# k-sheridan/mantis

Measured on AMD Instinct MI355X. Metric: poses/sec + p50 per-frame latency, 1280x720 4-cam batch, higher is better.
Workload: dtype f64; 1 GPU; config3: 4-cam 1280x720 rig, shared map, full mantis3 path per camera + joint rig Gauss-Newton; cams_per_rig=4, contexts_per_gpu=6, landmarks=720, parallelism=rig-data-parallel x1

## Files before the change

mantis_amd/csrc/api.hip:

```cpp
#include <hip/hip_runtime.h>
#ifndef MK_FC_THREADS
#define MK_FC_THREADS 256
#endif

#include <algorithm>
#include <atomic>
#include <cfloat>
#include <chrono>
#include <cmath>
#include <cstdio>
#include <cstdlib>
#include <cstring>
#include <mutex>
#include <sstream>
#include <string>
#include <thread>
#include <vector>

#include <rccl/rccl.h>

#include "kernels.hip"

using namespace mk;

// ... 66 lines not shown
      return MANTIS_ERR_DEVICE;                                                   \
    }                                                                             \
  } while (0)

struct Ctx {
  mantis_config cfg{};
  hipStream_t s = nullptr;
  hipStream_t s_copy = nullptr;
  hipEvent_t ev_gauss = nullptr;
  hipEvent_t ev_wait = nullptr;
  int spin_frames = 16;
  std::string err;
  uint64_t rng_state = 1;
  double* d_lm = nullptr;
  int nw = 0, nr = 0, ng = 0;
  int F = 0, Wmax = 0, Hmax = 0;
  int n_cu = 256;
  bool trace_lds_ok = false;
  size_t trace_lds_max = 0;
  int trace_lds_frames = 0;
  int fc_small_frames = 0;
  size_t plane = 0;
  int pool_cap = 0;
  uint16_t* d_lroot = nullptr;
  size_t lstride = 0;
  size_t fstride = 0;
  uint8_t *d_bgr = nullptr, *d_strong = nullptr, *d_edge = nullptr,
          *d_det = nullptr, *d_mask = nullptr;
  int32_t* d_lab = nullptr;
  uint32_t *d_eb = nullptr, *d_b1 = nullptr, *d_b2 = nullptr;
// ... 83 lines not shown
  int gauss_cap = 0;
  RigWJob* d_rwjobs = nullptr;
  double* d_rwout = nullptr;
  size_t rw_cap = 0;
  int rw_rigs = 0, rw_C = 0;
  std::vector<double> rw_weights, rw_c2w, rw_sums;
  std::vector<int32_t> rw_chosen;
  bool has_prior = false;
  double prior_Twb[16];
  double* d_markov = nullptr;
  MarkovOp* d_mops = nullptr;
  int markov_n = 0;
  int32_t* d_agree = nullptr;
  bool agreed_fail = false;
  struct CallGraph {
    int n = 0, W = 0, H = 0, live = 0, nw = 0, nr = 0, ng = 0;
    bool vec = false;
    const void* lm = nullptr;
    const void* gauss = nullptr;
    hipGraphExec_t pre = nullptr, post = nullptr;
  };
  std::vector<CallGraph> graphs;
  bool use_graphs = false;
  bool screen_off = false;
  std::vector<std::pair<Cam, ScreenCam>> scam_cache;
  struct Track {
    void* d_in = nullptr;
    void* h_in = nullptr;
    size_t in_cap = 0;
    void* d_state = nullptr;
    void* d_res = nullptr;
// ... 62 lines not shown
  const bool mismatch = v[1] != -v[2];
  c->agreed_fail = v[0] != 0 || mismatch;
  if (local != MANTIS_OK) return local;
  if (v[0]) {
    c->err = "another rank of the communicator failed before this exchange (see its mantis_last_error)";
    return MANTIS_ERR_COMM;
  }
  if (mismatch) {
    c->err = "ranks passed different frame counts to a batched exchange (every rank must pass the same n_frames)";
    return MANTIS_ERR_ARG;
  }
  return MANTIS_OK;
}

inline Landmarks lmk_of(const Ctx* c) {
  return Landmarks{c->d_lm, c->nw, c->nr, c->ng, c->d_lm ? (const float4*)(c->d_lm + kLmfOffset) : nullptr};
}

void mark(Ctx* c, const char* name) {
  if (!c->prof) return;
  if (c->ev.size() <= c->ev_names.size()) {
    hipEvent_t e;
    (void)hipEventCreate(&e);
    c->ev.push_back(e);
  }
  (void)hipEventRecord(c->ev[c->ev_names.size()], c->s);
  c->ev_names.push_back(name);
}

struct Ctx;
hipError_t wait_stream(Ctx* c, int frames);
// ... 440 lines not shown
  if (ei != hipSuccess) {
    *out = nullptr;
    c->err = std::string("hipGraphInstantiate: ") + hipGetErrorString(ei);
    return MANTIS_ERR_DEVICE;
  }
  return MANTIS_OK;
}

Ctx::CallGraph* call_graph(Ctx* c, int n, int W, int H, const Shard* sh) {
  if (!c->use_graphs || sh || c->prof || n > c->fc_small_frames) return nullptr;
  const size_t hr_lds = (size_t)((H + HR_ROWS - 1) / HR_ROWS) * HR_ROWS * bits::words(W) * sizeof(uint32_t);
  if (!(c->hyst_rec && bits::words(W) <= 63 && H <= HR_ROWS * HR_MAXW && hr_lds <= c->hyst_rec_lds)) return nullptr;
  const int live = std::max(1, g_live_ctx[c->cfg.device & 63].load());
  for (auto& g : c->graphs)
    if (g.n == n && g.W == W && g.H == H && g.vec == c->vec_ok && g.live == live && g.lm == c->d_lm &&
        g.nw == c->nw && g.nr == c->nr && g.ng == c->ng && g.gauss == c->d_gauss)
      return &g;
  if (c->graphs.size() >= 8) {
    if (c->graphs.front().pre) (void)hipGraphExecDestroy(c->graphs.front().pre);
    if (c->graphs.front().post) (void)hipGraphExecDestroy(c->graphs.front().post);
    c->graphs.erase(c->graphs.begin());
  }
  Ctx::CallGraph g;
  g.n = n; g.W = W; g.H = H; g.vec = c->vec_ok; g.live = live;
  g.lm = c->d_lm; g.nw = c->nw; g.nr = c->nr; g.ng = c->ng; g.gauss = c->d_gauss;
  c->graphs.push_back(g);
  return &c->graphs.back();
}

mantis_status process_frames(Ctx* c, const mantis_image* cams, int n, const Shard* sh = nullptr) {
  if (!c->d_lm) { c->err = "map not set (mantis_set_map)"; return MANTIS_ERR_STATE; }
  if (n <= 0 || n > c->F) { c->err = "frame count exceeds max_cams"; return MANTIS_ERR_ARG; }
  const int ng = sh ? sh->n_global : n;
  if ((int64_t)c->cfg.particles * c->cfg.iterations * 6 * ng > INT32_MAX) {
    c->err = "particles x iterations x 6 x frames (all rig cameras when sharded) exceeds 2^31 gaussians per call";
    return MANTIS_ERR_ARG;
  }
  if (mantis_status e = ensure_gauss(c, ng)) return e;
  struct Joiner {
    std::thread t;
// ... 410 lines not shown

mantis_status mantis_set_map(void* ctx, const double* white, int32_t nw, const double* red, int32_t nr,
                             const double* green, int32_t ng) {
  Ctx* c = (Ctx*)ctx;
  if (c) bind_device(c);
  if (!c || nw < 0 || nr < 0 || ng < 0 || nw + nr + ng > 768 || ng > 64 || (nw && !white) || (nr && !red) ||
      (ng && !green)) {
    if (c) c->err = "map: need nw+nr+ng <= 768 and ng <= 64";
    return MANTIS_ERR_ARG;
  }
  std::vector<double> all;
  all.insert(all.end(), white, white + 3 * nw);
  all.insert(all.end(), red, red + 3 * nr);
  all.insert(all.end(), green, green + 3 * ng);
  const size_t nl = (size_t)nw + nr + ng;
  std::vector<double> buf(kLmfOffset + 2 * 768, 0.0);
  std::copy(all.begin(), all.end(), buf.begin());
  float* lf = (float*)(buf.data() + kLmfOffset);
  for (size_t i = 0; i < nl; i++) screen_landmark(all.data() + 3 * i, lf + 4 * i);
  if (c->d_lm) (void)hipFree(c->d_lm);
  c->d_lm = nullptr;
  if (dalloc(c, &c->d_lm, buf.size()) != MANTIS_OK) return MANTIS_ERR_OOM;
  HIP_OK(hipMemcpy(c->d_lm, buf.data(), sizeof(double) * buf.size(), hipMemcpyHostToDevice));
  c->nw = nw;
  c->nr = nr;
  c->ng = ng;
  c->h_lm = all;
  c->rf.pitch = 0;
  c->rf.rigs = 0;
  return MANTIS_OK;
}

int32_t mantis_parse_coordinates(const char* s, double* xyz, int32_t max_pts) {
  if (!s) return 0;
  std::vector<std::string> rows;
  std::stringstream ts(s);
  std::string tmp;
  while (std::getline(ts, tmp, ';')) {
    tmp.erase(std::remove(tmp.begin(), tmp.end(), '\n'), tmp.end());
    tmp.erase(std::remove(tmp.begin(), tmp.end(), ' '), tmp.end());
    rows.push_back(tmp);
// ... 766 lines not shown
```

mantis_amd/csrc/hostcheck.cpp:

```cpp
#include <algorithm>
#include <cstdint>
#include <cstring>
#include <vector>

static int g_jacobi_ff = 1;
#define MK_JACOBI_FF g_jacobi_ff
#include "mk_bits.h"
#include "mk_contour.h"
#include "mk_gn.h"
#include "mk_math.h"
#include "mk_mcl.h"
#include "mk_mcl_color.h"
#include "mk_mcl_modes.h"
#include "mk_refine.h"
#include "mk_rpp.h"
#include "mk_screen.h"
#include "mk_shard.h"
#include "mk_sort.h"
#include "mk_track.h"

extern "C" {

void hc_set_jacobi_ff(int on) { g_jacobi_ff = on; }

// ... 264 lines not shown
    const bool in = rp[2] > 0 && mk::in_frame(u, v, H, W);
    float xl[4];
    mk::screen_landmark(X + 3 * i, xl);
    int px = 0, py = 0;
    const int st = mk::screen_project(mk::posef_from(T), xl[0], xl[1], xl[2], xl[3], sc, W, H, &px, &py);
    res[4 * i] = st;
    res[4 * i + 1] = in;
    res[4 * i + 2] = st == mk::SCR_IN ? px : (in ? mk::cv_round(u) : 0);
    res[4 * i + 3] = st == mk::SCR_IN ? py : (in ? mk::cv_round(v) : 0);
    if ((st == mk::SCR_IN && (!in || px != mk::cv_round(u) || py != mk::cv_round(v))) || (st == mk::SCR_OUT && in))
      bad++;
  }
  return bad;
}

int hc_sizeof_cam_result(void) { return (int)sizeof(mantis_cam_result); }
int hc_sizeof_result(void) { return (int)sizeof(mantis_result); }
int hc_sizeof_shard_rec(void) { return (int)sizeof(mk::shard::Rec); }
void hc_shard_global_indices(int n_rigs, int n_local, const int32_t* cam_index, int cams_per_rig, int32_t* gidx) {
  mk::shard::global_indices(n_rigs, n_local, cam_index, cams_per_rig, gidx);
}
void hc_shard_pack_pairs(const int32_t* gidx, const int32_t* pf, int n_local, int slots, int32_t* pairs) {
  mk::shard::pack_pairs(gidx, pf, n_local, slots, pairs);
}
int64_t hc_shard_offsets(const int32_t* pairs, int npairs, int ng, int64_t per, int32_t* flags, int64_t* offset) {
  return mk::shard::offsets_from_pairs(pairs, npairs, ng, per, flags, offset);
}
void hc_shard_make_recs(const mantis_cam_result* res, const double* Tbc, const int32_t* gidx, int n, int slots,
                        mk::shard::Rec* out) {
  for (int s = 0; s < slots; s++) {
// ... 230 lines not shown
```

mantis_amd/csrc/kernels.hip:

```cpp
#include <hip/hip_runtime.h>

#include <cfloat>
#include <cstdint>
#include <type_traits>

#include "mk_bits.h"
#include "mk_contour.h"
#include "mk_gn.h"
#include "mk_math.h"
#include "mk_rpp.h"
#include "mk_shard.h"
#include "mk_sort.h"
#include "mk_track.h"
#include "mk_types.h"
#include "synth.h"

namespace mk {

#ifndef MK_DPP_SCAN
#define MK_DPP_SCAN 1
#endif
__device__ inline int wave_incl_scan(int v, int lane) {
#if MK_DPP_SCAN
  (void)lane;
// ... 3512 lines not shown
  for (int w = 0; w < wave; w++) base += wsum[w];
  int acc = base + incl - mine;
  for (int f = f0; f < f1; f++) {
    flags[ng + f] = acc;
    if (flags[f]) acc += per_frame;
  }
  if (t == 1023) *total = bad ? -1 : base + incl;
  __syncthreads();
  for (int f = t; f < n_local; f += 1024) st[f].gauss_offset = flags[ng + gidx[f]];
}

struct Landmarks {
  const double* xyz;
  int32_t nw, nr, ng;
  const float4* xyzf;
};
constexpr int kLmfOffset = 3 * 768;

struct MaskNone {
  __device__ uint32_t word(int, int, int) const { return 1u; }
  __device__ bool test(uint32_t, int) const { return true; }
};
struct MaskBytes {
  const uint8_t* m;
  __device__ uint32_t word(int lin, int, int) const { return m[lin]; }
  __device__ bool test(uint32_t w, int) const { return w != 0; }
};
typedef __attribute__((address_space(3))) const uint32_t lds_cu32;
struct MaskLds {
  lds_cu32* m;
  int Hp;
  __device__ uint32_t word(int, int x, int y) const { return m[__umul24((uint32_t)(x >> 5), (uint32_t)Hp) + y]; }
// ... 110 lines not shown
        if (cl->ok[l]) {
          total += (double)cl->acc[l] / (double)(10 * 10);
          n++;
        }
    }
    __builtin_amdgcn_wave_barrier();
    __threadfence_block();
  }
  if (lane == 0) {
    *n_out = n;
    *err_out = n <= 0 ? DBL_MAX : total / ((double)n * 1.1);
  }
}

constexpr int kColorPairs = 3072;
struct ColorPairs {
  int32_t x0[kColorPairs];
  int32_t yf[kColorPairs];
  int32_t acc[kColorPairs];
};
__device__ __attribute__((noinline)) int color_row_exact(const Xf& T, const double* X, const Cam& cm,
                                                         const uint8_t* bgr, int W, int H, int r) {
  double rp[3], u, v;
  xf_apply(T, X, rp);
  distort(cm, rp[0], rp[1], rp[2], &u, &v);
  const long npx = (long)W * H;
  const int y = cv_round(v + (-5.0 + (double)r));
  int rs = 0;
  for (int ox = 0; ox < 10; ox++) {
    const int x = cv_round(u + (-5.0 + (double)ox));
    const long lin = (long)y * W + x;
    int b = 0, g = 0, rr = 0;
    if (lin >= 0 && lin < npx) {
      const uint32_t pv = load_bgr(bgr, lin, npx);
// ... 19 lines not shown
    double rp[3], u, v;
    xf_apply(pose_of(h), green + 3 * l, rp);
    distort(cm, rp[0], rp[1], rp[2], &u, &v);
    const int ok = rp[2] > 0 && in_frame(u, v, H, W);
    const int x0 = cv_round(u + (-5.0 + 0.0)), y0 = cv_round(v + (-5.0 + 0.0));
    int xrun = 1, yrun = 1;
#pragma unroll
    for (int k = 1; k < 10; k++) {
      xrun &= cv_round(u + (-5.0 + (double)k)) == x0 + k;
      yrun &= cv_round(v + (-5.0 + (double)k)) == y0 + k;
    }
    cp->x0[i] = x0;
    cp->yf[i] = (int32_t)((uint32_t)y0 << 3) | (yrun << 2) | (xrun << 1) | ok;
    cp->acc[i] = 0;
  }
  __syncthreads();
  MK_CTICK(0);
  const int ni = 10 * np;
  constexpr int kU = 4;
  for (int q0 = tid; q0 < ni; q0 += kU * NT) {
    int rsum[kU], slot[kU];
#pragma unroll
    for (int k = 0; k < kU; k++) {
      const int q = q0 + k * NT;
      slot[k] = -1;
      rsum[k] = 0;
      if (q >= ni) continue;
      const int r = q / np, i = q - r * np;
      const int yf = cp->yf[i];
      if (!(yf & 1)) continue;
      slot[k] = i;
      const int x0 = cp->x0[i], y = (yf >> 3) + r;
      const long lin0 = (long)y * W + x0;
      if ((yf & 6) == 6 && lin0 >= 0 && lin0 + 12 <= npx) {
        rsum[k] = color_row_run(bgr, lin0);
      } else if ((yf & 6) == 6) {
        int rs = 0;
        for (int ox = 0; ox < 10; ox++) {
          const long lin = lin0 + ox;
          int b = 0, g = 0, rr = 0;
          if (lin >= 0 && lin < npx) {
            const uint32_t pv = load_bgr(bgr, lin, npx);
            b = (int)(pv & 0xffu);
            g = (int)((pv >> 8) & 0xffu);
            rr = (int)((pv >> 16) & 0xffu);
// ... 7 lines not shown
        rsum[k] = color_row_exact(pose_of(h), green + 3 * (i - h * ngr), cm, bgr, W, H, r);
      }
    }
#pragma unroll
    for (int k = 0; k < kU; k++)
      if (slot[k] >= 0) atomicAdd(&cp->acc[slot[k]], rsum[k]);
  }
  __syncthreads();
  MK_CTICK(1);
  for (int h = tid; h < nh; h += NT) {
    double total = 0;
    int n = 0;
    for (int l = 0; l < ngr; l++) {
      const int i = h * ngr + l;
      if (cp->yf[i] & 1) {
        total += (double)cp->acc[i] / (double)(10 * 10);
        n++;
      }
    }
    err[h] = n <= 0 ? DBL_MAX : total / ((double)n * 1.1);
  }
  __syncthreads();
}

#ifndef MK_SCR_UNROLL
#define MK_SCR_UNROLL 6
#endif
constexpr int kScrUnroll = MK_SCR_UNROLL;
struct UQueue {
  uint32_t* e;
  int32_t* n;
// ... 66 lines not shown
      const uint32_t off = hit ? l3 - 1u : 0u;
      typedef __attribute__((address_space(1), aligned(1))) const uint32_t gu32u;
      pv[k] = *(gu32u*)(gbytes(bgr) + off);
    }
#pragma unroll
    for (int k = 0; k < U; k++) asm volatile("" : "+v"(pv[k]));
    int cu = 0;
#pragma unroll
    for (int k = 0; k < U; k++) {
      cu += st[k] == SCR_UNSURE;
      const uint32_t d = ~(pv[k] >> 8) & 0xffffffu;
      const int term = (int)__builtin_amdgcn_udot4(d, d, 0u, false);
      constexpr int kBlack = 3 * 255 * 255;
      const int e = kBlack ^ ((term ^ kBlack) & hm[k]);
      const int im = st[k] == SCR_IN ? -1 : 0;
      n -= im;
      s += e & im;
    }
    if (__ballot(cu > 0)) {
      const int incl = wave_incl_scan(cu, lane);
      int base = 0;
      if (lane == 63) base = atomicAdd(q.n, incl);
      base = __builtin_amdgcn_readlane(base, 63);
      int idx = base + incl - cu;
#pragma unroll
      for (int k = 0; k < U; k++) {
        if (st[k] != SCR_UNSURE) continue;
        const int l = b0 + lane + 64 * k;
        if (idx < q.cap) {
          q.e[idx] = ((uint32_t)tag << 16) | (uint32_t)l;
        } else {
          int e;
          if (exact_term(*Tx, lmd + 3 * l, *cmp, W, H, bgr, mask, e)) { n++; s += e; }
        }
        idx++;
      }
    }
  }
  s_out = wave_sum(s);
  n_out = wave_sum(n);
}
template <int U, class MK>
__device__ inline void wave_sums_screen(const PoseF& P, const float4* lmf, int lb, int le, const ScreenCam& sc, int W,
                                        int H, const uint8_t* bgr, const MK& mask, UQueue q, int tag, const Xf* Tx,
                                        const double* lmd, const Cam* cmp, long long& s_out, int& n_out) {
  wave_sums_screen_t<U>(P, [&](int, int l) { return lmf[l]; }, lb, le, sc, W, H, bgr, mask, q, tag, Tx, lmd, cmp,
                        s_out, n_out);
}
template <int U>
struct WaveLms {
  float4 L[U];
  int lb, le;
  __device__ void load(const float4* lmf, int lb_, int le_) {
    lb = lb_;
    le = le_;
    const int lane = threadIdx.x & 63;
#pragma unroll
    for (int k = 0; k < U; k++) {
      const int l = lb + lane + 64 * k;
      L[k] = lmf[l < le ? l : le - 1];
    }
  }
  template <class MK>
  __device__ void sums(const PoseF& P, const ScreenCam& sc, int W, int H, const uint8_t* bgr, const MK& mask, UQueue q,
                       int tag, const Xf* Tx, const double* lmd, const Cam* cmp, long long& s_out, int& n_out) const {
    wave_sums_screen_t<U>(P, [&](int k, int) { return L[k]; }, lb, le, sc, W, H, bgr, mask, q, tag, Tx, lmd, cmp, s_out,
                          n_out);
  }
};

struct ScoreSlots {
  unsigned long long* s;
  int32_t* n;
};
template <int NT, int SPLIT, class MK>
struct BlockScore {
  static_assert((NT / 64) % SPLIT == 0 && 64 * kScrUnroll * SPLIT >= 768, "one register trip per slice");
  const FrameDesc& fd;
  const Cam* cmp;
  const double* lmd;
  const MK& mask;
  UQueue q;
  WaveLms<kScrUnroll> wl;
  __device__ void load(const float4* lmf, int nl) {
    const int h = (threadIdx.x >> 6) % SPLIT;
    wl.load(lmf, nl * h / SPLIT, nl * (h + 1) / SPLIT);
  }
};
struct StagedPoses {
  const PoseF* f;
  const Xf* c;
  __device__ const PoseF& pf(int j) const { return f[j]; }
  __device__ const Xf& c2w(int j) const { return c[j]; }
};
template <int NT, int SPLIT, class MK, class Poses>
__device__ __forceinline__ void block_score_tasks(const BlockScore<NT, SPLIT, MK>& b, const Poses& poses, int np,
                                                  ScoreSlots out) {
  const int wave = threadIdx.x >> 6, lane = threadIdx.x & 63;
  for (int task = __builtin_amdgcn_readfirstlane(wave); task < np * SPLIT; task += NT / 64) {
    const int j = task / SPLIT;
    long long s;
    int n;
    b.wl.sums(poses.pf(j), b.fd.scam, b.fd.w, b.fd.h, b.fd.bgr, b.mask, b.q, j, &poses.c2w(j), b.lmd, b.cmp, s, n);
    if (lane == 0) {
      atomicAdd(&out.s[j], (unsigned long long)s);
      atomicAdd(&out.n[j], n);
    }
  }
}
template <int NT, int SPLIT, class MK, class Poses>
__device__ __forceinline__ void block_score_drain(const BlockScore<NT, SPLIT, MK>& b, const Poses& poses,
                                                  ScoreSlots out) {
  const int n = min(*b.q.n, b.q.cap);
  for (int i = threadIdx.x; i < n; i += blockDim.x) {
    const uint32_t en = b.q.e[i];
    const int tag = (int)(en >> 16), l = (int)(en & 0xffffu);
    int e;
    if (exact_term(poses.c2w(tag), b.lmd + 3 * l, *b.cmp, b.fd.w, b.fd.h, b.fd.bgr, b.mask, e)) {
      atomicAdd(&out.s[tag], (unsigned long long)e);
      atomicAdd(&out.n[tag], 1);
    }
  }
}
template <int NT, int SPLIT, class MK, class Poses>
__device__ __forceinline__ void block_score(const BlockScore<NT, SPLIT, MK>& b, const Poses& poses, int np,
                                            ScoreSlots out) {
  block_score_tasks(b, poses, np, out);
  __syncthreads();
  block_score_drain(b, poses, out);
  __syncthreads();
}

template <class ErrOf>
__device__ __forceinline__ void wave_argmin(int np, const ErrOf& err_of, double& be, int& bj, int32_t& bn) {
  be = DBL_MAX;
// ... 141 lines not shown
    S.ctr = 0;
  }
  __syncthreads();
}

template <int NT>
__global__ __launch_bounds__(NT) void k_score_init(
    const FrameDesc* __restrict__ frames, const uint32_t* __restrict__ mbits, size_t bstride, Landmarks lmk,
    FrameState* st, HypRec* __restrict__ hyps, mantis_cam_result* __restrict__ res, FrameDebug* dbg,
    ScoreState* __restrict__ sst) {
  const int f = blockIdx.x;
  const int tid = threadIdx.x;
  const FrameDesc fd = frames[f];
  const MaskBits mask{mbits + (size_t)f * bstride, bits::tiled_rows(fd.h), fd.w};
  FrameDebug& D = dbg[f];
  const int nl = lmk.nw + lmk.nr + lmk.ng;
  __shared__ float4 lmf[768];
  __shared__ ErrIdx ei[kMaxHyps];
  __shared__ unsigned long long hs[kMaxHyps];
  __shared__ int32_t hn[kMaxHyps];
  __shared__ uint32_t uqe[kInitQueue];
  __shared__ int32_t uqn;
  __shared__ PoseLds cur;
  __shared__ int32_t nsc, uniq_bi;
  constexpr int kInitPoses = 128;
  __shared__ PoseF pfi[kInitPoses];
  if (!st[f].reaches_pf) {
    if (tid == 0) score_early_result(st[f], res[f], D);
    return;
  }
  for (int i = tid; i < nl; i += blockDim.x) lmf[i] = lmk.xyzf[i];
  __syncthreads();
  BlockScore<NT, 2, MaskBits> b{fd, &frames[f].cam, lmk.xyz, mask, UQueue{uqe, &uqn, kInitQueue}};
  b.load(lmf, nl);
  block_score_init<NT>(b, hyps + (size_t)f * kMaxHyps, st[f].n_hyps, D, ei, hs, hn, pfi, kInitPoses, cur, nsc, uniq_bi,
                       sst[f]);
}

__device__ inline void shift_values(int grid_size, double grid_spacing, double* shv) {
  double x = -((double)grid_size / 2.0) * grid_spacing + ((double)grid_spacing / 2.0);
  int k = 0;
  for (; x < ((double)grid_size / 2.0) * grid_spacing && k < 9; x += grid_spacing) shv[k++] = x;
}
__device__ inline void shift_pose(const Xf& w2c, const double* shv, int j, PoseLds& o) {
  Xf nw = w2c;
  nw.t[0] += shv[j / 9];
  nw.t[1] += shv[j % 9];
  nw.t[2] += 0.0;
// ... 42 lines not shown
    if (init && tid == 0) score_early_result(st[f], res[f], dbg[f]);
    return;
  }
  const FrameDesc fd = frames[f];
  const int W = fd.w, H = fd.h;
  const uint32_t* fm = mbits + (size_t)f * bstride;
  extern __shared__ __align__(16) uint32_t pf_mask[];
  if (LM) {
    typedef unsigned int u32x4 __attribute__((ext_vector_type(4)));
    const int n4 = (int)(bits::tiled_words(W, H) / 4);
    const u32x4* src = (const u32x4*)fm;
    u32x4* dst = (u32x4*)pf_mask;
    for (int i = tid; i < n4; i += NT) dst[i] = src[i];
  }
  FrameDebug& D = dbg[f];
  const int nl = lmk.nw + lmk.nr + lmk.ng;
  __shared__ PfLds<SPLIT> L;
  constexpr int kPfBuf = PfLds<SPLIT>::kBuf;
  float4* lmf = L.lmf;
  Xf *Pc = L.p.Pc, *Pw = L.p.Pw;
  PoseF* Pf = L.p.Pf;
  const ScoreSlots slots{L.p.Ps, L.p.Pn};
  int32_t& uqn = L.uqn;
  Xf &cur_c2w = L.cur_c2w, &cur_w2c = L.cur_w2c;
  double& cur_err = L.cur_err;
  for (int i = tid; i < nl; i += blockDim.x) lmf[i] = lmk.xyzf[i];
  if (tid == 0 && !init) {
    cur_c2w = sst[f].cur.c2w;
    cur_w2c = sst[f].cur.w2c;
    cur_err = sst[f].cur.err;
  }
// ... 5 lines not shown
  if (tid == 0) {                                  \
    const uint64_t nw = wall_clock64();            \
    tka[k] += (int32_t)(nw - tkp);                 \
    tkp = nw;                                      \
  }
#else
#define MK_PTICK(k)
#endif
  MK_PTICK(0);
  const float* gs = gauss + st[f].gauss_offset;
  using PfMask = typename std::conditional<LM, MaskLds, MaskBits>::type;
  const auto mask = [&] {
    if constexpr (LM) return MaskLds{(lds_cu32*)pf_mask, bits::tiled_rows(H)};
    else return MaskBits{fm, bits::tiled_rows(H), W};
  }();
  BlockScore<NT, SPLIT, PfMask> b{fd, &frames[f].cam, lmk.xyz, mask, UQueue{L.uqe, &L.uqn, kPfQueue}};
  b.load(lmf, nl);
  const StagedPoses poses{Pf, Pc};
  if (init) {
    static_assert(SPLIT == 2, "the init tasks use landmark halves");
    PoseLds& icur = L.icur;
    const int C = st[f].n_hyps;
    HypRec* Hh = hyps + (size_t)f * kMaxHyps;
    constexpr int kPer = (int)(sizeof(ErrIdx) + sizeof(unsigned long long) + sizeof(int32_t));
    const auto run = [&](unsigned char* buf) {
      ErrIdx* ei = (ErrIdx*)buf;
      unsigned long long* hs = (unsigned long long*)(ei + C);
      int32_t* hn = (int32_t*)(hs + C);
      block_score_init<NT>(b, Hh, C, D, ei, hs, hn, nullptr, 0, icur, L.insc, L.iuniq, sst[f]);
    };
    if (C * kPer <= kPfBuf && init != 2) run(L.init);
// ... 103 lines not shown
    sst[f].psum[tid] = (long long)slots.s[tid];
    sst[f].pcnt[tid] = slots.n[tid];
  }
}

template <int NT, int SPLIT>
__global__ __launch_bounds__(NT) void k_score_pf_part(
    const FrameDesc* __restrict__ frames, const uint32_t* __restrict__ mbits, size_t bstride, Landmarks lmk,
    const FrameState* __restrict__ st, const float* __restrict__ gauss, mantis_cam_result* __restrict__ res,
    FrameDebug* dbg, ScoreState* __restrict__ sst, int particles, int iterations, int it, int ppb, int nblk) {
  const int f = blockIdx.y, b = blockIdx.x;
  const int tid = threadIdx.x, wave = tid >> 6, lane = tid & 63;
  if (!st[f].reaches_pf) return;
  const FrameDesc fd = frames[f];
  const int W = fd.w, H = fd.h;
  const int nl = lmk.nw + lmk.nr + lmk.ng;
  constexpr int kW = NT / 64, kPP = kW / SPLIT > 0 ? kW / SPLIT : 1;
  __shared__ float4 lmf[768];
  __shared__ Xf Pc[kPP];
  __shared__ PoseF Pf[kPP];
  __shared__ unsigned long long Ps[kPP];
  __shared__ int32_t Pn[kPP];
  __shared__ uint32_t uqe[kPfQueue];
  __shared__ int32_t uqn, last;
  ScoreState& S = sst[f];
  const int p0 = b * ppb, np = max(0, min(ppb, particles - p0));
  const float* gs = gauss + st[f].gauss_offset + (size_t)it * particles * 6;
  for (int i = tid; i < nl; i += NT) lmf[i] = lmk.xyzf[i];
  if (tid < np) {
    Xf w2c, c2w;
    pf_particle(S.cur.w2c, gs + (size_t)(p0 + tid) * 6, w2c, c2w);
    Pc[tid] = c2w;
    Pf[tid] = posef_from(c2w);
    Ps[tid] = 0;
    Pn[tid] = 0;
  }
  if (tid == 0) uqn = 0;
  __syncthreads();
  const MaskBits mask{mbits + (size_t)f * bstride, bits::tiled_rows(H), W};
  BlockScore<NT, SPLIT, MaskBits> bs{fd, &frames[f].cam, lmk.xyz, mask, UQueue{uqe, &uqn, kPfQueue}};
  bs.load(lmf, nl);
  block_score(bs, StagedPoses{Pf, Pc}, np, ScoreSlots{Ps, Pn});
  if (tid < np) {
    S.psum[p0 + tid] = (long long)Ps[tid];
    S.pcnt[p0 + tid] = Pn[tid];
  }
  __threadfence();
  __syncthreads();
  if (tid == 0) last = atomicAdd(&S.ctr, 1) == nblk - 1;
  __syncthreads();
  if (!last || wave != 0) return;
  __threadfence();
  const volatile long long* vs = S.psum;
  const volatile int32_t* vc = S.pcnt;
  double be;
// ... 24 lines not shown
    }
  }
}

template <int NT, int SPLIT>
__device__ __forceinline__ void pose_score_block(const FrameDesc* __restrict__ frames,
                                                 const uint32_t* __restrict__ mbits, size_t bstride,
                                                 const Landmarks& lmk, const Xf* __restrict__ c2w,
                                                 const PoseF* __restrict__ pf, long long* __restrict__ sums,
                                                 int32_t* __restrict__ cnt, size_t t0, int C, int f, int cam,
                                                 int chunk, int np) {
  const int tid = threadIdx.x;
  constexpr int kPP = NT / 64 / SPLIT;
  static_assert(kPP >= 1, "a wave per slice");
  const FrameDesc fd = frames[f];
  const int nl = lmk.nw + lmk.nr + lmk.ng;
  __shared__ float4 lmf[768];
  __shared__ Xf Pc[kPP];
  __shared__ PoseF Pf[kPP];
  __shared__ unsigned long long Ps[kPP];
  __shared__ int32_t Pn[kPP];
  __shared__ uint32_t uqe[kPfQueue];
  __shared__ int32_t uqn;
  const int j0 = chunk * kPP, nj = max(0, min(kPP, np - j0));
  for (int i = tid; i < nl; i += NT) lmf[i] = lmk.xyzf[i];
  if (tid < nj) {
    const size_t t = t0 + (size_t)(j0 + tid) * C + cam;
    Pc[tid] = c2w[t];
    Pf[tid] = pf[t];
    Ps[tid] = 0;
    Pn[tid] = 0;
  }
  if (tid == 0) uqn = 0;
  __syncthreads();
  const MaskBits mask{mbits + (size_t)f * bstride, bits::tiled_rows(fd.h), fd.w};
  BlockScore<NT, SPLIT, MaskBits> b{fd, &frames[f].cam, lmk.xyz, mask, UQueue{uqe, &uqn, kPfQueue}};
  b.load(lmf, nl);
  block_score(b, StagedPoses{Pf, Pc}, nj, ScoreSlots{Ps, Pn});
  if (tid < nj) {
    const size_t t = t0 + (size_t)(j0 + tid) * C + cam;
    sums[t] = (long long)Ps[tid];
    cnt[t] = Pn[tid];
  }
}

struct ShiftPoses {
  const PoseLds* P;
  __device__ PoseF pf(int j) const { return posef_from(P[j].c2w); }
  __device__ const Xf& c2w(int j) const { return P[j].c2w; }
};
template <int NT>
__global__ __launch_bounds__(NT) void k_score_shift_part(
    const FrameDesc* __restrict__ frames, const uint32_t* __restrict__ mbits, size_t bstride, Landmarks lmk,
    const FrameState* __restrict__ st, ScoreState* __restrict__ sst, double grid_spacing, int grid_size, int spb) {
  const int f = blockIdx.y, b = blockIdx.x;
  const int tid = threadIdx.x, wave = tid >> 6, lane = tid & 63;
  if (!st[f].reaches_pf) return;
  const FrameDesc fd = frames[f];
  const int W = fd.w, H = fd.h;
  const MaskBits mask{mbits + (size_t)f * bstride, bits::tiled_rows(H), W};
  const int nl = lmk.nw + lmk.nr + lmk.ng;
  constexpr int NS = 81, kMaxSpb = NT / 128 > 0 ? NT / 128 : 1;
  __shared__ float4 lmf[768];
  __shared__ PoseLds P[kMaxSpb];
  __shared__ double shv[9];
  __shared__ unsigned long long hs[kMaxSpb];
  __shared__ int32_t hn[kMaxSpb];
  __shared__ uint32_t uqe[kTailQueue];
  __shared__ int32_t uqn;
  const int j0 = b * spb, ns = max(0, min(min(spb, kMaxSpb), NS - j0));
  for (int i = tid; i < nl; i += NT) lmf[i] = lmk.xyzf[i];
  if (tid == 0) {
    uqn = 0;
    shift_values(grid_size, grid_spacing, shv);
  }
  __syncthreads();
  if (tid < ns) {
    shift_pose(sst[f].cur.w2c, shv, j0 + tid, P[tid]);
    hs[tid] = 0;
    hn[tid] = 0;
  }
  __syncthreads();
  BlockScore<NT, 2, MaskBits> bs{fd, &frames[f].cam, lmk.xyz, mask, UQueue{uqe, &uqn, kTailQueue}};
  bs.load(lmf, nl);
  block_score(bs, ShiftPoses{P}, ns, ScoreSlots{hs, hn});
  if (tid < ns) {
    sst[f].psum[j0 + tid] = (long long)hs[tid];
    sst[f].pcnt[j0 + tid] = hn[tid];
  }
}

template <int NT>
__global__ __launch_bounds__(NT) void k_score_final(
    const FrameDesc* __restrict__ frames, Landmarks lmk, const FrameState* __restrict__ st,
    mantis_cam_result* __restrict__ res, FrameDebug* dbg, const ScoreState* __restrict__ sst, double grid_spacing,
    int grid_size) {
  const int f = blockIdx.x;
  const int tid = threadIdx.x, wave = tid >> 6, lane = tid & 63;
// ... 223 lines not shown
#ifndef MK_DENSE_HYPS
#define MK_DENSE_HYPS 64
#endif
constexpr int kApiHyps = 16, kApiQueue = 1024, kDenseHyps = MK_DENSE_HYPS;
struct ApiPoses {
  const PoseF* f;
  const double* c;
  __device__ const PoseF& pf(int j) const { return f[j]; }
  __device__ const Xf& c2w(int j) const { return *(const Xf*)(c + 12 * (size_t)j); }
};
template <int HPB, class MK>
__device__ inline void score_api_fast(const FrameDesc& fd, const Cam* cmp, const MK& mask, Landmarks lmk,
                                      const double* c2w, int n, double* err, int32_t* nproj) {
  const int tid = threadIdx.x;
  const int h0 = blockIdx.x * HPB, nh = min(HPB, n - h0);
  const int nl = lmk.nw + lmk.nr + lmk.ng;
  __shared__ float4 lmf[768];
  __shared__ unsigned long long hs[HPB];
  __shared__ int32_t hn[HPB];
  __shared__ uint32_t uqe[kApiQueue];
  __shared__ int32_t uqn;
  __shared__ PoseF pf[HPB];
  for (int i = tid; i < nl; i += blockDim.x) lmf[i] = lmk.xyzf[i];
  for (int i = tid; i < HPB; i += blockDim.x) {
    hs[i] = 0;
    hn[i] = 0;
    if (i < nh) pf[i] = posef_from(*(const Xf*)(c2w + 12 * (size_t)(h0 + i)));
  }
  if (tid == 0) uqn = 0;
  __syncthreads();
  BlockScore<64 * kApiHyps, 2, MK> b{fd, cmp, lmk.xyz, mask, UQueue{uqe, &uqn, kApiQueue}};
  b.load(lmf, nl);
  block_score(b, ApiPoses{pf, c2w + 12 * (size_t)h0}, nh, ScoreSlots{hs, hn});
  for (int i = tid; i < nh; i += blockDim.x) {
    err[h0 + i] = track::error_of((long long)hs[i], hn[i]);
    nproj[h0 + i] = hn[i];
  }
}
__global__ __launch_bounds__(64 * kApiHyps) void k_score_api(const FrameDesc* __restrict__ frames, const uint8_t* mask,
                                                             Landmarks lmk, const double* __restrict__ c2w, int n,
                                                             int fast, double* __restrict__ err,
                                                             int32_t* __restrict__ nproj) {
  const FrameDesc fd = frames[0];
  if (fast) {
    if (mask) score_api_fast<kApiHyps>(fd, &frames[0].cam, MaskBytes{mask}, lmk, c2w, n, err, nproj);
    else score_api_fast<kApiHyps>(fd, &frames[0].cam, MaskNone{}, lmk, c2w, n, err, nproj);
// ... 29 lines not shown
```

mantis_amd/csrc/mk_screen.h:

```cpp
#pragma once
#include <cmath>
#include <cstdint>

#include "mk_math.h"

namespace mk {

struct ScreenCam {
  float fx, fy, cx, cy;
  float k[4];
  float sens;
  float crel;
  float c2, e0;
};
struct PoseF {
  float R[9];
  float t[3];
  float tn;
  float pad[3];
};

constexpr float kScrU = 5.9604644775390625e-8f;
enum { SCR_OUT = 0, SCR_IN = 1, SCR_UNSURE = 2 };

// ... 99 lines not shown
  const bool outside = (int)((unsigned)iu > (unsigned)W) | (int)((unsigned)iv > (unsigned)H);
  const bool sure = (int)valid & (int)round_ok & (int)interior;
  const bool out = (int)(z < -ez) | ((int)valid & (int)outside);
  *px = iu;
  *py = iv;
  return sure ? SCR_IN : (out ? SCR_OUT : SCR_UNSURE);
}

MK_HD void screen_landmark(const double* X, float* o) {
  o[0] = (float)X[0];
  o[1] = (float)X[1];
  o[2] = (float)X[2];
  o[3] = (float)((fabs(X[0]) + fabs(X[1]) + fabs(X[2])) * (6.0 * 5.9604644775390625e-8) * 1.000001);
}

struct ScreenBounds {
  double S, M;
  bool ok;
};
MK_HD ScreenBounds screen_bounds(const double* k, int pieces = 4096) {
  ScreenBounds r{1.0, 1.0, true};
  const double half_pi = 1.5707963267948966;
  for (int i = 0; i < pieces; i++) {
    const double a = half_pi * i / pieces, b = fmin(half_pi, half_pi * (i + 1) / pieces * (1 + 1e-15));
    const double xa = a * a, xb = b * b;
    double dhi = 1, dlo = 1, Fhi = 1, Flo = 1, Ahi = 0, pa = xa, pb = xb;
    for (int j = 0; j < 4; j++) {
      const double ta = k[j] * pa, tb = k[j] * pb;
      const double mx = fmax(ta, tb), mn = fmin(ta, tb);
      dhi += (2 * j + 3) * mx;
// ... 36 lines not shown
```

Before: 30790 rig poses/s.

## Deduplicate identical map landmarks and colour sample pairs, weighting scores by multiplicity

When the map is set, identical landmark coordinates are collapsed on the host into a distinct list. Each landmark's multiplicity is packed into the low mantissa bits of its screening-tolerance float, and every scoring kernel iterates only the distinct landmarks, adding weight×error and weight to the sums. The colour-row stage builds an LDS hash table so duplicate pixel pairs are sampled once and their result is shared. Scoring also dispatches to an unroll depth matched to the actual number of landmark slots. This removes redundant projection and pixel work when the map repeats points, at the cost of a quadratic host dedup and a slightly inflated screening tolerance.

New measurement: 31490 rig poses/s (median of 5 runs). 2.3% higher.

```diff
diff --git a/mantis_amd/csrc/api.hip b/mantis_amd/csrc/api.hip
--- a/mantis_amd/csrc/api.hip
+++ b/mantis_amd/csrc/api.hip
@@ -104,6 +104,7 @@
   uint64_t rng_state = 1;
   double* d_lm = nullptr;
   int nw = 0, nr = 0, ng = 0;
+  int nd = 0;
   int F = 0, Wmax = 0, Hmax = 0;
   int n_cu = 256;
   bool trace_lds_ok = false;
@@ -217,7 +218,7 @@
   int32_t* d_agree = nullptr;
   bool agreed_fail = false;
   struct CallGraph {
-    int n = 0, W = 0, H = 0, live = 0, nw = 0, nr = 0, ng = 0;
+    int n = 0, W = 0, H = 0, live = 0, nw = 0, nr = 0, ng = 0, nd = 0;
     bool vec = false;
     const void* lm = nullptr;
     const void* gauss = nullptr;
@@ -310,7 +311,8 @@
 }
 
 inline Landmarks lmk_of(const Ctx* c) {
-  return Landmarks{c->d_lm, c->nw, c->nr, c->ng, c->d_lm ? (const float4*)(c->d_lm + kLmfOffset) : nullptr};
+  return Landmarks{c->d_lm, c->nw, c->nr, c->ng, c->d_lm ? (const float4*)(c->d_lm + kLmfOffset) : nullptr,
+                   c->d_lm ? c->d_lm + kLmdOffset : nullptr, c->nd};
 }
 
 void mark(Ctx* c, const char* name) {
@@ -781,7 +783,7 @@
   const int live = std::max(1, g_live_ctx[c->cfg.device & 63].load());
   for (auto& g : c->graphs)
     if (g.n == n && g.W == W && g.H == H && g.vec == c->vec_ok && g.live == live && g.lm == c->d_lm &&
-        g.nw == c->nw && g.nr == c->nr && g.ng == c->ng && g.gauss == c->d_gauss)
+        g.nw == c->nw && g.nr == c->nr && g.ng == c->ng && g.nd == c->nd && g.gauss == c->d_gauss)
       return &g;
   if (c->graphs.size() >= 8) {
     if (c->graphs.front().pre) (void)hipGraphExecDestroy(c->graphs.front().pre);
@@ -790,7 +792,7 @@
   }
   Ctx::CallGraph g;
   g.n = n; g.W = W; g.H = H; g.vec = c->vec_ok; g.live = live;
-  g.lm = c->d_lm; g.nw = c->nw; g.nr = c->nr; g.ng = c->ng; g.gauss = c->d_gauss;
+  g.lm = c->d_lm; g.nw = c->nw; g.nr = c->nr; g.ng = c->ng; g.nd = c->nd; g.gauss = c->d_gauss;
   c->graphs.push_back(g);
   return &c->graphs.back();
 }
@@ -1231,10 +1233,12 @@
   all.insert(all.end(), red, red + 3 * nr);
   all.insert(all.end(), green, green + 3 * ng);
   const size_t nl = (size_t)nw + nr + ng;
-  std::vector<double> buf(kLmfOffset + 2 * 768, 0.0);
+  std::vector<double> buf(kLmdOffset + 3 * 768, 0.0);
   std::copy(all.begin(), all.end(), buf.begin());
+  std::vector<int32_t> wt(nl + 1);
+  const int nd = distinct_landmarks(all.data(), (int)nl, buf.data() + kLmdOffset, wt.data());
   float* lf = (float*)(buf.data() + kLmfOffset);
-  for (size_t i = 0; i < nl; i++) screen_landmark(all.data() + 3 * i, lf + 4 * i);
+  for (int i = 0; i < nd; i++) screen_landmark_w(buf.data() + kLmdOffset + 3 * i, wt[i], lf + 4 * i);
   if (c->d_lm) (void)hipFree(c->d_lm);
   c->d_lm = nullptr;
   if (dalloc(c, &c->d_lm, buf.size()) != MANTIS_OK) return MANTIS_ERR_OOM;
@@ -1242,6 +1246,7 @@
   c->nw = nw;
   c->nr = nr;
   c->ng = ng;
+  c->nd = nd;
   c->h_lm = all;
   c->rf.pitch = 0;
   c->rf.rigs = 0;
diff --git a/mantis_amd/csrc/hostcheck.cpp b/mantis_amd/csrc/hostcheck.cpp
--- a/mantis_amd/csrc/hostcheck.cpp
+++ b/mantis_amd/csrc/hostcheck.cpp
@@ -302,6 +302,15 @@
   return bad;
 }
 
+int hc_distinct_landmarks(const double* xyz, int n, double* dxyz, int32_t* w, float* rec, int32_t* wrec) {
+  const int nd = mk::distinct_landmarks(xyz, n, dxyz, w);
+  for (int i = 0; i < nd; i++) {
+    mk::screen_landmark_w(dxyz + 3 * i, w[i], rec + 4 * i);
+    wrec[i] = mk::screen_landmark_weight(rec[4 * i + 3]);
+  }
+  return nd;
+}
+
 int hc_sizeof_cam_result(void) { return (int)sizeof(mantis_cam_result); }
 int hc_sizeof_result(void) { return (int)sizeof(mantis_result); }
 int hc_sizeof_shard_rec(void) { return (int)sizeof(mk::shard::Rec); }
diff --git a/mantis_amd/csrc/kernels.hip b/mantis_amd/csrc/kernels.hip
--- a/mantis_amd/csrc/kernels.hip
+++ b/mantis_amd/csrc/kernels.hip
@@ -3550,8 +3550,11 @@
   const double* xyz;
   int32_t nw, nr, ng;
   const float4* xyzf;
+  const double* dxyz;
+  int32_t nd;
 };
 constexpr int kLmfOffset = 3 * 768;
+constexpr int kLmdOffset = kLmfOffset + 2 * 768;
 
 struct MaskNone {
   __device__ uint32_t word(int, int, int) const { return 1u; }
@@ -3692,10 +3695,15 @@
 }
 
 constexpr int kColorPairs = 3072;
+constexpr int kColorHash = 8192;
 struct ColorPairs {
   int32_t x0[kColorPairs];
   int32_t yf[kColorPairs];
   int32_t acc[kColorPairs];
+  uint16_t rep[kColorPairs];
+  uint16_t list[kColorPairs];
+  int32_t nlist, nok;
+  int32_t tab[kColorHash];
 };
 __device__ __attribute__((noinline)) int color_row_exact(const Xf& T, const double* X, const Cam& cm,
                                                          const uint8_t* bgr, int W, int H, int r) {
@@ -3745,9 +3753,32 @@
     cp->yf[i] = (int32_t)((uint32_t)y0 << 3) | (yrun << 2) | (xrun << 1) | ok;
     cp->acc[i] = 0;
   }
+  for (int i = tid; i < kColorHash; i += NT) cp->tab[i] = -1;
+  if (tid == 0) cp->nlist = cp->nok = 0;
+  __syncthreads();
+  for (int i = tid; i < np; i += NT) {
+    const int yf = cp->yf[i];
+    if (!(yf & 1)) continue;
+    if (ctk) atomicAdd(&cp->nok, 1);
+    const int x0 = cp->x0[i];
+    int r = i;
+    if ((yf & 6) == 6) {
+      uint32_t s = ((uint32_t)x0 * 0x9E3779B1u + (uint32_t)yf * 0x85EBCA77u) >> 19;
+      static_assert(kColorHash == 1 << 13, "hash bits");
+      for (;; s = (s + 1) & (kColorHash - 1)) {
+        const int o = atomicCAS(&cp->tab[s], -1, i);
+        if (o < 0) break;
+        if (cp->x0[o] == x0 && cp->yf[o] == yf) { r = o; break; }
+      }
+    }
+    cp->rep[i] = (uint16_t)r;
+    if (r == i) cp->list[atomicAdd(&cp->nlist, 1)] = (uint16_t)i;
+  }
   __syncthreads();
   MK_CTICK(0);
-  const int ni = 10 * np;
+  if (ctk && tid == 0) ctk[0] = cp->nok << 16 | cp->nlist;
+  const int nl = cp->nlist;
+  const int ni = 10 * nl;
   constexpr int kU = 4;
   for (int q0 = tid; q0 < ni; q0 += kU * NT) {
     int rsum[kU], slot[kU];
@@ -3757,9 +3788,8 @@
       slot[k] = -1;
       rsum[k] = 0;
       if (q >= ni) continue;
-      const int r = q / np, i = q - r * np;
+      const int r = q / nl, i = cp->list[q - r * nl];
       const int yf = cp->yf[i];
-      if (!(yf & 1)) continue;
       slot[k] = i;
       const int x0 = cp->x0[i], y = (yf >> 3) + r;
       const long lin0 = (long)y * W + x0;
@@ -3797,7 +3827,7 @@
     for (int l = 0; l < ngr; l++) {
       const int i = h * ngr + l;
       if (cp->yf[i] & 1) {
-        total += (double)cp->acc[i] / (double)(10 * 10);
+        total += (double)cp->acc[cp->rep[i]] / (double)(10 * 10);
         n++;
       }
     }
@@ -3894,8 +3924,10 @@
       constexpr int kBlack = 3 * 255 * 255;
       const int e = kBlack ^ ((term ^ kBlack) & hm[k]);
       const int im = st[k] == SCR_IN ? -1 : 0;
-      n -= im;
-      s += e & im;
+      const int l = b0 + lane + 64 * k;
+      const int w = screen_landmark_weight(lm_at(k, l < le ? l : le - 1).w);
+      n += w & im;
+      s += (int)__umul24((uint32_t)(e & im), (uint32_t)w);
     }
     if (__ballot(cu > 0)) {
       const int incl = wave_incl_scan(cu, lane);
@@ -3911,7 +3943,11 @@
           q.e[idx] = ((uint32_t)tag << 16) | (uint32_t)l;
         } else {
           int e;
-          if (exact_term(*Tx, lmd + 3 * l, *cmp, W, H, bgr, mask, e)) { n++; s += e; }
+          if (exact_term(*Tx, lmd + 3 * l, *cmp, W, H, bgr, mask, e)) {
+            const int w = screen_landmark_weight(lm_at(k, l).w);
+            n += w;
+            s += w * e;
+          }
         }
         idx++;
       }
@@ -3938,13 +3974,14 @@
 #pragma unroll
     for (int k = 0; k < U; k++) {
       const int l = lb + lane + 64 * k;
-      L[k] = lmf[l < le ? l : le - 1];
-    }
-  }
-  template <class MK>
+      L[k] = lmf[max(l < le ? l : le - 1, 0)];
+    }
+  }
+  __device__ int slots() const { return (le - lb + 63) >> 6; }
+  template <int K, class MK>
   __device__ void sums(const PoseF& P, const ScreenCam& sc, int W, int H, const uint8_t* bgr, const MK& mask, UQueue q,
                        int tag, const Xf* Tx, const double* lmd, const Cam* cmp, long long& s_out, int& n_out) const {
-    wave_sums_screen_t<U>(P, [&](int k, int) { return L[k]; }, lb, le, sc, W, H, bgr, mask, q, tag, Tx, lmd, cmp, s_out,
+    wave_sums_screen_t<K>(P, [&](int k, int) { return L[k]; }, lb, le, sc, W, H, bgr, mask, q, tag, Tx, lmd, cmp, s_out,
                           n_out);
   }
 };
@@ -3959,6 +3996,7 @@
   const FrameDesc& fd;
   const Cam* cmp;
   const double* lmd;
+  const float4* lmw;
   const MK& mask;
   UQueue q;
   WaveLms<kScrUnroll> wl;
@@ -3973,20 +4011,37 @@
   __device__ const PoseF& pf(int j) const { return f[j]; }
   __device__ const Xf& c2w(int j) const { return c[j]; }
 };
-template <int NT, int SPLIT, class MK, class Poses>
-__device__ __forceinline__ void block_score_tasks(const BlockScore<NT, SPLIT, MK>& b, const Poses& poses, int np,
-                                                  ScoreSlots out) {
+template <int K, int NT, int SPLIT, class MK, class Poses>
+__device__ __forceinline__ void block_score_tasks_k(const BlockScore<NT, SPLIT, MK>& b, const Poses& poses, int np,
+                                                    ScoreSlots out) {
   const int wave = threadIdx.x >> 6, lane = threadIdx.x & 63;
   for (int task = __builtin_amdgcn_readfirstlane(wave); task < np * SPLIT; task += NT / 64) {
     const int j = task / SPLIT;
     long long s;
     int n;
-    b.wl.sums(poses.pf(j), b.fd.scam, b.fd.w, b.fd.h, b.fd.bgr, b.mask, b.q, j, &poses.c2w(j), b.lmd, b.cmp, s, n);
+    b.wl.template sums<K>(poses.pf(j), b.fd.scam, b.fd.w, b.fd.h, b.fd.bgr, b.mask, b.q, j, &poses.c2w(j), b.lmd, b.cmp,
+                          s, n);
     if (lane == 0) {
       atomicAdd(&out.s[j], (unsigned long long)s);
       atomicAdd(&out.n[j], n);
     }
   }
+}
+template <int K, int NT, int SPLIT, class MK, class Poses>
+__device__ __forceinline__ void block_score_tasks_n(const BlockScore<NT, SPLIT, MK>& b, const Poses& poses, int np,
+                                                    ScoreSlots out, int ns) {
+  if constexpr (K > 1) {
+    if (ns < K) {
+      block_score_tasks_n<K - 1>(b, poses, np, out, ns);
+      return;
+    }
+  }
+  block_score_tasks_k<K>(b, poses, np, out);
+}
+template <int NT, int SPLIT, class MK, class Poses>
+__device__ __forceinline__ void block_score_tasks(const BlockScore<NT, SPLIT, MK>& b, const Poses& poses, int np,
+                                                  ScoreSlots out) {
+  block_score_tasks_n<kScrUnroll>(b, poses, np, out, __builtin_amdgcn_readfirstlane(b.wl.slots()));
 }
 template <int NT, int SPLIT, class MK, class Poses>
 __device__ __forceinline__ void block_score_drain(const BlockScore<NT, SPLIT, MK>& b, const Poses& poses,
@@ -3997,8 +4052,9 @@
     const int tag = (int)(en >> 16), l = (int)(en & 0xffffu);
     int e;
     if (exact_term(poses.c2w(tag), b.lmd + 3 * l, *b.cmp, b.fd.w, b.fd.h, b.fd.bgr, b.mask, e)) {
-      atomicAdd(&out.s[tag], (unsigned long long)e);
-      atomicAdd(&out.n[tag], 1);
+      const int w = screen_landmark_weight(b.lmw[l].w);
+      atomicAdd(&out.s[tag], (unsigned long long)(w * e));
+      atomicAdd(&out.n[tag], w);
     }
   }
 }
@@ -4170,7 +4226,7 @@
   const FrameDesc fd = frames[f];
   const MaskBits mask{mbits + (size_t)f * bstride, bits::tiled_rows(fd.h), fd.w};
   FrameDebug& D = dbg[f];
-  const int nl = lmk.nw + lmk.nr + lmk.ng;
+  const int nl = lmk.nd;
   __shared__ float4 lmf[768];
   __shared__ ErrIdx ei[kMaxHyps];
   __shared__ unsigned long long hs[kMaxHyps];
@@ -4187,7 +4243,7 @@
   }
   for (int i = tid; i < nl; i += blockDim.x) lmf[i] = lmk.xyzf[i];
   __syncthreads();
-  BlockScore<NT, 2, MaskBits> b{fd, &frames[f].cam, lmk.xyz, mask, UQueue{uqe, &uqn, kInitQueue}};
+  BlockScore<NT, 2, MaskBits> b{fd, &frames[f].cam, lmk.dxyz, lmk.xyzf, mask, UQueue{uqe, &uqn, kInitQueue}};
   b.load(lmf, nl);
   block_score_init<NT>(b, hyps + (size_t)f * kMaxHyps, st[f].n_hyps, D, ei, hs, hn, pfi, kInitPoses, cur, nsc, uniq_bi,
                        sst[f]);
@@ -4260,7 +4316,7 @@
     for (int i = tid; i < n4; i += NT) dst[i] = src[i];
   }
   FrameDebug& D = dbg[f];
-  const int nl = lmk.nw + lmk.nr + lmk.ng;
+  const int nl = lmk.nd;
   __shared__ PfLds<SPLIT> L;
   constexpr int kPfBuf = PfLds<SPLIT>::kBuf;
   float4* lmf = L.lmf;
@@ -4296,7 +4352,7 @@
     if constexpr (LM) return MaskLds{(lds_cu32*)pf_mask, bits::tiled_rows(H)};
     else return MaskBits{fm, bits::tiled_rows(H), W};
   }();
-  BlockScore<NT, SPLIT, PfMask> b{fd, &frames[f].cam, lmk.xyz, mask, UQueue{L.uqe, &L.uqn, kPfQueue}};
+  BlockScore<NT, SPLIT, PfMask> b{fd, &frames[f].cam, lmk.dxyz, lmk.xyzf, mask, UQueue{L.uqe, &L.uqn, kPfQueue}};
   b.load(lmf, nl);
   const StagedPoses poses{Pf, Pc};
   if (init) {
@@ -4430,7 +4486,7 @@
   if (!st[f].reaches_pf) return;
   const FrameDesc fd = frames[f];
   const int W = fd.w, H = fd.h;
-  const int nl = lmk.nw + lmk.nr + lmk.ng;
+  const int nl = lmk.nd;
   constexpr int kW = NT / 64, kPP = kW / SPLIT > 0 ? kW / SPLIT : 1;
   __shared__ float4 lmf[768];
   __shared__ Xf Pc[kPP];
@@ -4454,7 +4510,7 @@
   if (tid == 0) uqn = 0;
   __syncthreads();
   const MaskBits mask{mbits + (size_t)f * bstride, bits::tiled_rows(H), W};
-  BlockScore<NT, SPLIT, MaskBits> bs{fd, &frames[f].cam, lmk.xyz, mask, UQueue{uqe, &uqn, kPfQueue}};
+  BlockScore<NT, SPLIT, MaskBits> bs{fd, &frames[f].cam, lmk.dxyz, lmk.xyzf, mask, UQueue{uqe, &uqn, kPfQueue}};
   bs.load(lmf, nl);
   block_score(bs, StagedPoses{Pf, Pc}, np, ScoreSlots{Ps, Pn});
   if (tid < np) {
@@ -4509,7 +4565,7 @@
   constexpr int kPP = NT / 64 / SPLIT;
   static_assert(kPP >= 1, "a wave per slice");
   const FrameDesc fd = frames[f];
-  const int nl = lmk.nw + lmk.nr + lmk.ng;
+  const int nl = lmk.nd;
   __shared__ float4 lmf[768];
   __shared__ Xf Pc[kPP];
   __shared__ PoseF Pf[kPP];
@@ -4529,7 +4585,7 @@
   if (tid == 0) uqn = 0;
   __syncthreads();
   const MaskBits mask{mbits + (size_t)f * bstride, bits::tiled_rows(fd.h), fd.w};
-  BlockScore<NT, SPLIT, MaskBits> b{fd, &frames[f].cam, lmk.xyz, mask, UQueue{uqe, &uqn, kPfQueue}};
+  BlockScore<NT, SPLIT, MaskBits> b{fd, &frames[f].cam, lmk.dxyz, lmk.xyzf, mask, UQueue{uqe, &uqn, kPfQueue}};
   b.load(lmf, nl);
   block_score(b, StagedPoses{Pf, Pc}, nj, ScoreSlots{Ps, Pn});
   if (tid < nj) {
@@ -4554,7 +4610,7 @@
   const FrameDesc fd = frames[f];
   const int W = fd.w, H = fd.h;
   const MaskBits mask{mbits + (size_t)f * bstride, bits::tiled_rows(H), W};
-  const int nl = lmk.nw + lmk.nr + lmk.ng;
+  const int nl = lmk.nd;
   constexpr int NS = 81, kMaxSpb = NT / 128 > 0 ? NT / 128 : 1;
   __shared__ float4 lmf[768];
   __shared__ PoseLds P[kMaxSpb];
@@ -4576,7 +4632,7 @@
     hn[tid] = 0;
   }
   __syncthreads();
-  BlockScore<NT, 2, MaskBits> bs{fd, &frames[f].cam, lmk.xyz, mask, UQueue{uqe, &uqn, kTailQueue}};
+  BlockScore<NT, 2, MaskBits> bs{fd, &frames[f].cam, lmk.dxyz, lmk.xyzf, mask, UQueue{uqe, &uqn, kTailQueue}};
   bs.load(lmf, nl);
   block_score(bs, ShiftPoses{P}, ns, ScoreSlots{hs, hn});
   if (tid < ns) {
@@ -4830,7 +4886,7 @@
                                       const double* c2w, int n, double* err, int32_t* nproj) {
   const int tid = threadIdx.x;
   const int h0 = blockIdx.x * HPB, nh = min(HPB, n - h0);
-  const int nl = lmk.nw + lmk.nr + lmk.ng;
+  const int nl = lmk.nd;
   __shared__ float4 lmf[768];
   __shared__ unsigned long long hs[HPB];
   __shared__ int32_t hn[HPB];
@@ -4845,7 +4901,7 @@
   }
   if (tid == 0) uqn = 0;
   __syncthreads();
-  BlockScore<64 * kApiHyps, 2, MK> b{fd, cmp, lmk.xyz, mask, UQueue{uqe, &uqn, kApiQueue}};
+  BlockScore<64 * kApiHyps, 2, MK> b{fd, cmp, lmk.dxyz, lmk.xyzf, mask, UQueue{uqe, &uqn, kApiQueue}};
   b.load(lmf, nl);
   block_score(b, ApiPoses{pf, c2w + 12 * (size_t)h0}, nh, ScoreSlots{hs, hn});
   for (int i = tid; i < nh; i += blockDim.x) {
diff --git a/mantis_amd/csrc/mk_screen.h b/mantis_amd/csrc/mk_screen.h
--- a/mantis_amd/csrc/mk_screen.h
+++ b/mantis_amd/csrc/mk_screen.h
@@ -1,6 +1,7 @@
 #pragma once
 #include <cmath>
 #include <cstdint>
+#include <cstring>
 
 #include "mk_math.h"
 
@@ -137,6 +138,32 @@
   o[3] = (float)((fabs(X[0]) + fabs(X[1]) + fabs(X[2])) * (6.0 * 5.9604644775390625e-8) * 1.000001);
 }
 
+constexpr int kLmWBits = 10;
+MK_HD void screen_landmark_w(const double* X, int w, float* o) {
+  screen_landmark(X, o);
+  const float xn = o[3] > 1e-30f ? o[3] : 1e-30f;
+  const uint32_t m = (1u << kLmWBits) - 1u;
+  uint32_t b = __builtin_bit_cast(uint32_t, xn);
+  b = ((b + m) & ~m) | ((uint32_t)(w - 1) & m);
+  o[3] = __builtin_bit_cast(float, b);
+}
+MK_HD int screen_landmark_weight(float xn) {
+  return (int)(__builtin_bit_cast(uint32_t, xn) & ((1u << kLmWBits) - 1u)) + 1;
+}
+inline int distinct_landmarks(const double* xyz, int n, double* dxyz, int32_t* w) {
+  int nd = 0;
+  for (int i = 0; i < n; i++) {
+    int j = 0;
+    while (j < nd && memcmp(dxyz + 3 * j, xyz + 3 * i, 3 * sizeof(double)) != 0) j++;
+    if (j == nd) {
+      memcpy(dxyz + 3 * nd, xyz + 3 * i, 3 * sizeof(double));
+      w[nd++] = 0;
+    }
+    w[j]++;
+  }
+  return nd;
+}
+
 struct ScreenBounds {
   double S, M;
   bool ok;
```
